# microsoft/EVA

Measured on AMD Instinct MI355X. Metric: homomorphic ops/sec (mul+rescale+relin) at N=2^16, L=10; execute() wall-time, higher is better.
Workload: dtype u64

## Files before the change

### eva_amd/csrc/internal.hip.h

```cpp
#pragma once
#include "../../include/eva_hip.h"

#include <hip/hip_runtime.h>

#include <algorithm>
#include <cmath>
#include <cstdlib>
#include <cstring>
#include <functional>
#include <map>
#include <memory>
#include <mutex>
#include <stdexcept>
#include <string>
#include <tuple>
#include <unordered_map>
#include <vector>

#include "devmath.hip.h"
#include "hostmath.h"

namespace evah {

extern thread_local std::string g_err;
// ... 36 lines not shown
    in_use += bytes;
    return p;
  }
  void free(void *p, size_t bytes) {
    bytes = (bytes + 255) & ~(size_t)255;
    free_[bytes].push_back(p);
    in_use -= bytes;
    cached += bytes;
  }
  void release_cached() {
    for (auto &kv : free_)
      for (void *p : kv.second) (void)hipFree(p);
    free_.clear();
    cached = 0;
  }
};

struct Buffer {
  u64 *d;
  size_t bytes;
  int refs;
  Pool *pool;
  evah_ctx *owner;
  bool ready_everywhere;
  std::vector<evah_ctx *> synced;
  std::vector<evah_ctx *> readers;
};

enum KClass {
  KC_EW = 0,
  KC_INTT_A,
  KC_INTT_B,
  KC_KSDIGIT_A,
  KC_KSDIGIT_B,
  KC_KSMAC,
  KC_MODDOWN_A,
  KC_MODDOWN_B,
  KC_NTT_A,
  KC_NTT_B,
  KC_COUNT
};
static const char *const kclass_names[KC_COUNT] = {
    "elementwise", "intt_pass1", "intt_pass2", "ksdigit_pass1", "ksdigit_pass2", "ks_mac",
    "moddown_pass1", "moddown_pass2", "ntt_pass1", "ntt_pass2"};

struct ProfRec {
  hipEvent_t e0, e1;
  int cls;
};

__host__ __device__ inline size_t keyp_block_words(uint32_t nd) { return ((size_t)2 * nd + 1) * 256; }
struct KeyDev {
  u64 *d = nullptr;
  uint32_t n_digits = 0;
  size_t bytes = 0;
  uint32_t rows = 0;
  u64 *d_split = nullptr;
  u64 *d_perm = nullptr;
};

}

using namespace evah;

struct evah_ct {
  Buffer *buf;
  u64 *d;
  uint32_t size, limbs;
  size_t ps;
  double scale;
  uint32_t batch = 1;
};
struct evah_pt {
  Buffer *buf;
  u64 *d;
  uint32_t limbs;
  double scale;
  bool uniform = false;
};
struct evah_graph {
  hipGraph_t graph = nullptr;
  hipGraphExec_t exec = nullptr;
  struct Reserved { evah_ctx *ctx; void *p; size_t bytes; };
  std::vector<Reserved> reserved;
};

struct SharedDev {
  int device = 0;
  void *d_tables = nullptr;
  KeyDev relin;
  KeyDev pk, sk;
  double2 *dec_roots = nullptr;
  std::map<uint32_t, KeyDev> galois;
  std::map<uint32_t, uint32_t *> perms;
  std::map<uint32_t, uint32_t *> perms_inv;
  std::map<uint32_t, u64 *> hoist_sign;
  std::map<std::pair<uint32_t, uint32_t>, u64 *> hoist_corr;
  double2 *enc_roots = nullptr;
  double enc_last_root[2] = {0, 0};
  uint32_t *enc_slot_map = nullptr;
  uint32_t key_rows = 0, key_shard = 0;
  uint64_t xfer[6] = {0, 0, 0, 0, 0, 0};
  ~SharedDev() {
    (void)hipSetDevice(device);
    if (enc_roots) (void)hipFree(enc_roots);
    if (enc_slot_map) (void)hipFree(enc_slot_map);
    if (relin.d) (void)hipFree(relin.d);
    if (relin.d_split) (void)hipFree(relin.d_split);
    if (pk.d) (void)hipFree(pk.d);
    if (sk.d) { (void)hipMemset(sk.d, 0, sk.bytes); (void)hipFree(sk.d); }
    if (dec_roots) (void)hipFree(dec_roots);
    for (auto &kv : galois) {
      (void)hipFree(kv.second.d);
      if (kv.second.d_split) (void)hipFree(kv.second.d_split);
      if (kv.second.d_perm) (void)hipFree(kv.second.d_perm);
    }
    for (auto &kv : perms) (void)hipFree(kv.second);
    for (auto &kv : perms_inv) (void)hipFree(kv.second);
    for (auto &kv : hoist_sign) (void)hipFree(kv.second);
    for (auto &kv : hoist_corr) (void)hipFree(kv.second);
    if (d_tables) (void)hipFree(d_tables);
  }
};

struct Tunables {
  bool fuse_mac = true;
  bool fuse_mul = true;
  bool fuse_mul2 = true;
  bool ew_fuse = true;
  bool ew_uniform = true;
  uint32_t fuse_small_blocks = 2048;
  int small_lr = 2;
  uint32_t small_lr_blocks = 1024;
  bool hoist = true;
  uint32_t hoist_min_tiles = 2048;
  bool hoist_debug = false;
  bool peer_self_check = false;
  bool hoist_table_fail = false;
  bool fuse_special_inv = true;
  int ks_groups = 1;
  int ks_threads = 64;
  bool fold_pa = true;
  bool win_fuse = true;
  bool win_linear = true;
  bool fb_persist = true;
  uint32_t fb_grid = 0;
  bool mac3 = true;
  uint32_t loop_n = 8, loop_min = 2, loop_min_wgs = 2048, loop_target_wgs = 8192;
  bool hoist_map = true;
  uint32_t hoist_v = 1;
  bool side_stream = false;
  bool chain_step = true, chain_batched = true;
  uint32_t chain_fuse_blocks = 256;
  uint32_t lds_extra = 0;

  static Tunables from_env(uint32_t N) {
    Tunables t;
    auto flag = [](const char *name, bool &v) { if (const char *e = std::getenv(name)) v = std::atoi(e) != 0; };
    auto count = [](const char *name, uint32_t &v) { if (const char *e = std::getenv(name)) v = (uint32_t)std::max(0, std::atoi(e)); };
    (void)N;
    flag("EVAH_FUSE_MAC", t.fuse_mac);
    flag("EVAH_FUSE_MUL", t.fuse_mul);
    flag("EVAH_FUSE_MUL2", t.fuse_mul2);
    flag("EVAH_EW_FUSE", t.ew_fuse);
    flag("EVAH_EW_UNIFORM", t.ew_uniform);
    count("EVAH_FUSE_SMALL", t.fuse_small_blocks);
    if (const char *e = std::getenv("EVAH_SMALL_LR")) t.small_lr = std::atoi(e) == 3 ? 3 : 2;
    count("EVAH_SMALL_LR_BLOCKS", t.small_lr_blocks);
    flag("EVAH_HOIST", t.hoist);
    count("EVAH_HOIST_MIN_TILES", t.hoist_min_tiles);
    flag("EVAH_HOIST_DEBUG", t.hoist_debug);
    flag("EVAH_HOIST_TABLE_FAIL", t.hoist_table_fail);
    flag("EVAH_PEER_SELF_CHECK", t.peer_self_check);
    flag("EVAH_FUSE_SPECIAL_INV", t.fuse_special_inv);
    flag("EVAH_FOLD_PA", t.fold_pa);
    flag("EVAH_WIN_FUSE", t.win_fuse);
    flag("EVAH_WIN_LINEAR", t.win_linear);
    flag("EVAH_FB_PERSIST", t.fb_persist);
    count("EVAH_FB_GRID", t.fb_grid);
    flag("EVAH_MAC3", t.mac3);
    count("EVAH_LOOP_N", t.loop_n);
    count("EVAH_LOOP_MIN", t.loop_min);
    count("EVAH_LOOP_MIN_WGS", t.loop_min_wgs);
    count("EVAH_LOOP_TARGET_WGS", t.loop_target_wgs);
    count("EVAH_LDS_EXTRA", t.lds_extra);
    flag("EVAH_HOIST_MAP", t.hoist_map);
    flag("EVAH_SIDE_STREAM", t.side_stream);
    flag("EVAH_CHAIN_STEP", t.chain_step);
    flag("EVAH_CHAIN_BATCHED", t.chain_batched);
    count("EVAH_CHAIN_FUSE_BLOCKS", t.chain_fuse_blocks);
    count("EVAH_HOIST_V", t.hoist_v);
    if (const char *e = std::getenv("EVAH_KS_GROUPS")) t.ks_groups = std::max(1, std::atoi(e));
    if (const char *e = std::getenv("EVAH_KS_THREADS")) {
      const int n = std::atoi(e);
      if (n == 64 || n == 128 || n == 256) t.ks_threads = n;
    }
    return t;
  }
};

struct evah_ctx {
  std::shared_ptr<SharedDev> sh;
  int device = 0;
  uint32_t N = 0, logN = 0, k = 0;
  std::vector<u64> primes;
  std::vector<int> total_bits;
  DevCtx dev{};
  hipStream_t own = nullptr, stream = nullptr;
  hipStream_t side = nullptr;
  Pool pool;
  hipEvent_t ev0 = nullptr, ev1 = nullptr;
  bool capturing = false;
  std::vector<hipEvent_t> capture_events;
  std::vector<hipEvent_t> sync_events;
  Tunables tun;
  bool all_tb = false;
  bool prof_on = false;
  std::vector<ProfRec> prof_recs;
  std::vector<hipEvent_t> prof_free;
  double prof_ms[KC_COUNT] = {0};
  uint64_t prof_n[KC_COUNT] = {0};
};

namespace evah {

inline void use(evah_ctx *c) { HIPCHK(hipSetDevice(c->device)); }
inline void count_h2d(evah_ctx *c, size_t bytes, bool plain = false) { c->sh->xfer[plain ? 2 : 0]++; c->sh->xfer[4] += bytes; }
inline void count_d2h(evah_ctx *c, size_t bytes, bool plain = false) { c->sh->xfer[plain ? 3 : 1]++; c->sh->xfer[5] += bytes; }

inline hipEvent_t prof_event(evah_ctx *c) {
  if (!c->prof_free.empty()) {
    hipEvent_t e = c->prof_free.back();
    c->prof_free.pop_back();
    return e;
  }
  hipEvent_t e;
  HIPCHK(hipEventCreate(&e));
  return e;
}
inline void prof_drain(evah_ctx *c) {
  for (auto &r : c->prof_recs) {
    float ms = 0;
    HIPCHK(hipEventSynchronize(r.e1));
    HIPCHK(hipEventElapsedTime(&ms, r.e0, r.e1));
    c->prof_ms[r.cls] += ms;
    c->prof_n[r.cls]++;
    c->prof_free.push_back(r.e0);
    c->prof_free.push_back(r.e1);
  }
  c->prof_recs.clear();
}
struct ProfScope {
  evah_ctx *c;
  int cls;
  hipEvent_t e0 = nullptr;
  ProfScope(evah_ctx *c_, int cls_) : c(c_), cls(cls_) {
    if (c->prof_on && !c->capturing) {
      if (c->prof_recs.size() >= 8192) prof_drain(c);
      e0 = prof_event(c);
      HIPCHK(hipEventRecord(e0, c->stream));
    }
  }
  ~ProfScope() {
    if (e0) {
      hipEvent_t e1 = prof_event(c);
      (void)hipEventRecord(e1, c->stream);
      c->prof_recs.push_back({e0, e1, cls});
    }
  }
};

inline Buffer *buf_new(evah_ctx *c, size_t elems) {
  Buffer *b = new Buffer;
  b->bytes = elems * sizeof(u64);
  b->d = (u64 *)c->pool.alloc(b->bytes);
  b->refs = 1;
  b->pool = &c->pool;
  b->owner = c;
  b->ready_everywhere = false;
  return b;
}
inline void h2d_now(evah_ctx *c, void *dst, const void *src, size_t bytes) {
  HIPCHK(hipMemcpyAsync(dst, src, bytes, hipMemcpyHostToDevice, c->stream));
  HIPCHK(hipStreamSynchronize(c->stream));
}
inline hipEvent_t sync_event(evah_ctx *c) {
  if (!c->capturing && !c->sync_events.empty()) {
    hipEvent_t e = c->sync_events.back();
    c->sync_events.pop_back();
    return e;
  }
  hipEvent_t e;
  HIPCHK(hipEventCreateWithFlags(&e, hipEventDisableTiming));
  return e;
}
inline void stream_wait(evah_ctx *waiter, evah_ctx *signaller) {
  if (waiter == signaller || waiter->stream == signaller->stream) return;
  if (waiter->sh.get() != signaller->sh.get()) {
    int cur = 0;
    HIPCHK(hipGetDevice(&cur));
    HIPCHK(hipSetDevice(signaller->device));
    hipEvent_t e = sync_event(signaller);
    hipError_t rc = hipEventRecord(e, signaller->stream);
    (void)hipSetDevice(waiter->device);
    if (rc == hipSuccess) rc = hipStreamWaitEvent(waiter->stream, e, 0);
    (void)hipSetDevice(cur);
    if (waiter->capturing || signaller->capturing) signaller->capture_events.push_back(e);
    else signaller->sync_events.push_back(e);
    HIPCHK(rc);
    return;
  }
  hipEvent_t e = sync_event(waiter);
  HIPCHK(hipEventRecord(e, signaller->stream));
  HIPCHK(hipStreamWaitEvent(waiter->stream, e, 0));
  if (waiter->capturing || signaller->capturing) waiter->capture_events.push_back(e);
  else waiter->sync_events.push_back(e);
}
struct SideStream {
  evah_ctx *c;
  hipStream_t main;
  bool forked = false, on_side = false;
  explicit SideStream(evah_ctx *c_) : c(c_), main(c_->stream) {}
  void link(hipStream_t from, hipStream_t to) {
    hipEvent_t e = sync_event(c);
    HIPCHK(hipEventRecord(e, from));
    HIPCHK(hipStreamWaitEvent(to, e, 0));
    if (c->capturing) c->capture_events.push_back(e);
    else c->sync_events.push_back(e);
  }
  void fork() {
    if (!c->side) HIPCHK(hipStreamCreateWithFlags(&c->side, hipStreamNonBlocking));
    link(main, c->side);
    c->stream = c->side;
    forked = on_side = true;
  }
  void back() { c->stream = main; on_side = false; }
  void join() {
    back();
    if (forked) link(c->side, main);
    forked = false;
  }
  ~SideStream() {
    c->stream = main;
// ... 108 lines not shown
```

### eva_amd/csrc/keyswitch.hip

```cpp
#include "launch.hip.h"

namespace evah {

__global__ void __launch_bounds__(256)
k_ks_mac(DevCtx cx, const u64 *target, const u64 *scratch, const u64 *key, u64 *prod, uint32_t l) {
  if (cx.skipped()) return;
  const uint32_t I = blockIdx.y;
  const uint32_t kap = (I == l) ? cx.k - 1 : I;
  const size_t n = 2 * ((size_t)blockIdx.x * blockDim.x + threadIdx.x);
  const DevPrime pm = cx.primes[kap];
  const size_t N = cx.N, key_digit = (size_t)2 * cx.k * N;
  u128_t a0x = {0, 0}, a0y = {0, 0}, a1x = {0, 0}, a1y = {0, 0};
  for (uint32_t J = 0; J < l; J++) {
    const u64 *op = (I == J) ? target + (size_t)J * N : scratch + ((size_t)I * l + J) * N;
    const ulonglong2 o = ld2(op + n);
    const u64 *kp = key + J * key_digit + (size_t)kap * N + n;
    const ulonglong2 k0 = ld2(kp), k1 = ld2(kp + (size_t)cx.k * N);
    acc128(a0x, o.x, k0.x);
    acc128(a0y, o.y, k0.y);
    acc128(a1x, o.x, k1.x);
    acc128(a1y, o.y, k1.y);
  }
  ulonglong2 r0, r1;
  r0.x = barrett128(a0x, pm);
  r0.y = barrett128(a0y, pm);
  r1.x = barrett128(a1x, pm);
  r1.y = barrett128(a1y, pm);
  st2(prod + (size_t)I * N + n, r0);
  st2(prod + ((size_t)(l + 1) + I) * N + n, r1);
}

template <int P, int LR>
static void launch_ks_inner_plr(evah_ctx *c, const u64 *target, const u64 *scratch, const KsBatch &kb, u64 *prod, uint32_t l) {
  ProfScope ps(c, KC_KSMAC);
  const uint32_t max_tile = (uint32_t)c->tun.ks_threads << LR;
  const uint32_t tile = c->N < max_tile ? c->N : max_tile;
  const int logC = (int)ilog2(tile) - P;
  if (logC < 0) throw std::runtime_error("ks_inner tile smaller than one sub-transform");
  const size_t lds = ((((size_t)1 << logC) * lds_sub_stride<P>() + 1) & ~(size_t)1) * sizeof(u64) +
                     ((size_t)1 << (logC + P)) * sizeof(ulonglong2) +
                     (kb.mac3 ? (size_t)tile * sizeof(u64) : 0);
  const uint32_t n_tiles = c->N / tile;
  auto go = [&](auto kernel, const auto &mt, const auto &at) {
    hipLaunchKernelGGL(kernel, dim3(n_tiles * kb.n, kb.ni), dim3(tile >> LR), lds, c->stream, c->dev, target, kb.target_bs, scratch,
                       kb.scratch_bs, kb.keys, prod, kb.prod_bs, l, kb.i0, logC, n_tiles, kb.n, kb.targets, mt, kb.istep,
                       kb.nout ? kb.nout : l + 1, kb.r_out, at, (kb.lazy_out ? 1 : 0) | (kb.diag ? 2 : 0), kb.fold_row);
  };
  if (kb.r_out && ((tile >> LR) > 64 || kb.istep != 1)) throw std::logic_error("fused special-row inverse pass needs the one-wave key-switch kernel");
  if (kb.fold && kb.istep != 1) throw std::logic_error("the folded key-switch forms are not used on limb shards");
  if (kb.fold && !kb.mul && !kb.adds) throw std::logic_error("folded key switch without polynomials to fold");
  const int mode = kb.mul ? (kb.fold ? KS_FOLDMUL : KS_MUL) : (kb.fold ? KS_FOLDADD : KS_PLAIN);
  auto with_mode = [&](auto mode_tag) {
    constexpr int M = decltype(mode_tag)::value;
    const KsMulArg<M> mt = [&] { if constexpr (M == KS_MUL || M == KS_FOLDMUL) return *kb.mul; else return NoMul{}; }();
    const KsAddArg<M> at = [&] { if constexpr (M == KS_FOLDADD) return *kb.adds; else return NoMul{}; }();
    if constexpr (M != KS_MUL) {
      if (kb.mac3 && (tile >> LR) <= 64) {
        if (kb.r_out) go(ks_inner_kernel<P, LR, 64, M, true, true>, mt, at);
        else go(ks_inner_kernel<P, LR, 64, M, false, true>, mt, at);
        return;
      }
    }
    if (kb.mac3) throw std::logic_error("split keys handed to a key-switch kernel that accumulates in 128 bits");
    if (kb.r_out) go(ks_inner_kernel<P, LR, 64, M, true>, mt, at);
    else if ((tile >> LR) <= 64) go(ks_inner_kernel<P, LR, 64, M>, mt, at);
    else go(ks_inner_kernel<P, LR, NTT_THREADS, M>, mt, at);
  };
  switch (mode) {
  case KS_PLAIN: with_mode(std::integral_constant<int, KS_PLAIN>{}); break;
  case KS_MUL: with_mode(std::integral_constant<int, KS_MUL>{}); break;
  case KS_FOLDMUL: with_mode(std::integral_constant<int, KS_FOLDMUL>{}); break;
  default: with_mode(std::integral_constant<int, KS_FOLDADD>{}); break;
  }
  HIPCHK(hipGetLastError());
}
template <int LR>
static void launch_ks_inner_lr(evah_ctx *c, int P, const u64 *target, const u64 *scratch, const KsBatch &key, u64 *prod, uint32_t l) {
  switch (P) {
  case 5: launch_ks_inner_plr<5, LR>(c, target, scratch, key, prod, l); break;
  case 6: launch_ks_inner_plr<6, LR>(c, target, scratch, key, prod, l); break;
  case 7: launch_ks_inner_plr<7, LR>(c, target, scratch, key, prod, l); break;
  case 8: launch_ks_inner_plr<8, LR>(c, target, scratch, key, prod, l); break;
  default: throw std::runtime_error("unsupported poly_modulus_degree for the key-switch kernel");
  }
}
void launch_ks_inner(evah_ctx *c, int P, const u64 *target, const u64 *scratch, const KsBatch &key, u64 *prod, uint32_t l) {
  launch_ks_inner_lr<2>(c, P, target, scratch, key, prod, l);
}

bool switch_key_products(evah_ctx *c, uint32_t l, const u64 *target, size_t target_bs, const KeyDev *const *keys,
                         uint32_t n, u64 *prod_d, const PtrTab *target_tab, const MulTab *mul, u64 *r_small, bool fold,
                         const PtrTab *adds, bool lazy_out) {
  const size_t N = c->N;
  if (n < 1 || n > (uint32_t)KS_BATCH_MAX) throw std::runtime_error("key-switch batch out of range");
  KsBatch kb;
  kb.n = n;
  kb.target_bs = target_bs;
  kb.scratch_bs = (size_t)(l + 1) * l * N;
  kb.prod_bs = (size_t)2 * (l + 1) * N;
  const uint32_t ks_tile = std::min<uint32_t>(c->N, (uint32_t)c->tun.ks_threads << 2);
  bool mac3 = c->tun.mac3 && c->tun.fuse_mac && c->all_tb && l <= 15 && (ks_tile >> 2) <= 64 && !(mul && !fold);
  for (uint32_t b = 0; b < n; b++) {
    if (keys[b]->n_digits < l) throw std::runtime_error("key switching key has too few digits");
    if (keys[b]->rows != c->k) throw std::logic_error("this context holds a limb shard's key rows: use the evah_shard_* entry points");
    mac3 = mac3 && keys[b]->d_split;
  }
  for (uint32_t b = 0; b < n; b++) kb.keys.key[b] = mac3 ? keys[b]->d_split : keys[b]->d;
  kb.mac3 = mac3;
  if (target_tab) kb.targets = *target_tab;
  kb.mul = mul;
  kb.fold = fold;
  kb.adds = adds;
  kb.lazy_out = lazy_out;
  if ((mul || fold) && !c->tun.fuse_mac) throw std::logic_error("the fused multiply / folded forms need the fused key-switch kernel");
  Scratch t(c, (size_t)n * l * N);
  Scratch sc(c, n * kb.scratch_bs);
  Scratch d2(c, mul && fold ? (size_t)n * l * N : 1);
  if (mul && fold) {
    target = d2.d;
    kb.target_bs = target_bs = (size_t)l * N;
  }
  OpKsDigit::Params dp{t.d, sc.d, l, (size_t)l * N, kb.scratch_bs, 0, l + 1};
  const bool small = c->tun.fuse_mac && std::max(1, c->tun.ks_groups) == 1 && fuse_small_launch(c, n * (l + 1) * l);
  if (mul) {
    OpMulIntt::Params ip{*mul, t.d, (size_t)l * N, l, fold ? d2.d : nullptr};
    if (small) launch_pass_p<false, true, OpMulIntt>(c, c->logN / 2, ip, n * l);
    else ntt_inverse<OpMulIntt>(c, ip, n * l);
  } else {
    OpPlain::Params ip{target, t.d, target_bs, (size_t)l * N, l, 0, 0, {}};
    if (target_tab) ip.src_tab = *target_tab;
    if (small) launch_pass_p<false, true, OpPlain>(c, c->logN / 2, ip, n * l);
    else ntt_inverse<OpPlain>(c, ip, n * l);
  }
  if (small) {
    dp.i0 = kb.i0 = 0;
    dp.ni = kb.ni = l + 1;
    launch_inv_fwd<OpKsDigit>(c, dp, n * (l + 1) * l);
    const uint32_t max_tile = (uint32_t)c->tun.ks_threads << 2;
    if (r_small && c->tun.fuse_special_inv && (std::min<uint32_t>(c->N, max_tile) >> 2) <= 64) kb.r_out = r_small;
    launch_ks_inner(c, c->logN / 2, target, sc.d, kb, prod_d, l);
    return kb.r_out != nullptr;
  }
  if (c->tun.fuse_mac) {
    const int a = (c->logN + 1) / 2, b = c->logN / 2;
    const uint32_t groups = std::min<uint32_t>(std::max(1, c->tun.ks_groups), l + 1);
    const uint32_t max_tile = (uint32_t)c->tun.ks_threads << 2;
    if (r_small && groups == 1 && c->tun.fuse_special_inv && (std::min<uint32_t>(c->N, max_tile) >> 2) <= 64) kb.r_out = r_small;
    for (uint32_t g = 0; g < groups; g++) {
      const uint32_t i0 = (uint32_t)((uint64_t)(l + 1) * g / groups), i1 = (uint32_t)((uint64_t)(l + 1) * (g + 1) / groups);
      if (i1 == i0) continue;
      dp.i0 = kb.i0 = i0;
      dp.ni = kb.ni = i1 - i0;
      launch_pass_p<true, false, OpKsDigit>(c, a, dp, n * (i1 - i0) * l);
      launch_ks_inner(c, b, target, sc.d, kb, prod_d, l);
    }
    return kb.r_out != nullptr;
  } else {
    ntt_forward<OpKsDigit>(c, dp, n * (l + 1) * l);
    for (uint32_t b = 0; b < n; b++) {
      ProfScope ps(c, KC_KSMAC);
      hipLaunchKernelGGL(k_ks_mac, dim3(c->N / 512, l + 1), dim3(256), 0, c->stream, c->dev,
                         target ? target + b * target_bs : target_tab->p[b], sc.d + b * kb.scratch_bs, keys[b]->d,
                         prod_d + b * kb.prod_bs, l);
      HIPCHK(hipGetLastError());
    }
  }
  return false;
}

void switch_key(evah_ctx *c, uint32_t l, const u64 *target, const KeyDev &key, const u64 *add,
                       size_t add_ps, uint32_t add_polys, u64 *out, size_t out_ps) {
  const size_t N = c->N;
  Scratch prod(c, (size_t)2 * (l + 1) * N);
  Scratch r(c, 2 * N);
  const KeyDev *kp = &key;
  const bool fold = c->tun.fold_pa && c->tun.fuse_mac && add && add_polys >= 1 && add_polys <= 2;
  PtrTab adds{};
  if (fold)
    for (uint32_t K = 0; K < add_polys; K++) adds.p[K] = add + K * add_ps;
  const bool inv1 = switch_key_products(c, l, target, 0, &kp, 1, prod.d, nullptr, nullptr, fuse_small_launch(c, 2 * l) ? r.d : nullptr,
                                        fold, fold ? &adds : nullptr);
  if (fold) add = nullptr;
  OpPlain::Params sp{prod.d + (size_t)l * N, r.d, (size_t)(l + 1) * N, N, 1, c->k - 1, 1, {}};
    OpModDown::Params mp{r.d, N, prod.d, (size_t)(l + 1) * N, add, add_ps, add_polys, out, out_ps,
                       c->k - 1, l};
  inverse_then_forward<OpPlain, OpModDown>(c, sp, 2, mp, 2 * l, inv1);
}

}

extern "C" {

int evah_relinearize(evah_ctx *c, const evah_ct *a, evah_ct **out) {
  API_BEGIN
  use(c);
  acquire(c, a->buf);
  if (a->size != 3) throw std::invalid_argument("relinearize expects a size-3 ciphertext");
  if (!c->sh->relin.d) throw std::invalid_argument("relinearization key not present");
  evah_ct *o = ct_new(c, 2, a->limbs, a->scale, a->batch);
  try {
    if (a->batch == 1) {
      switch_key(c, a->limbs, a->d + 2 * a->ps, c->sh->relin, a->d, a->ps, 2, o->d, o->ps);
    } else {
      const uint32_t l = a->limbs;
      const size_t N = c->N, pps = (size_t)(l + 1) * N;
      for (uint32_t b0 = 0; b0 < a->batch; b0 += KS_BATCH_MAX) {
        const uint32_t n = std::min<uint32_t>(KS_BATCH_MAX, a->batch - b0);
        const u64 *a0 = a->d + (size_t)b0 * 3 * a->ps;
        Scratch prod(c, (size_t)n * 2 * pps);
        std::vector<const KeyDev *> keys(n, &c->sh->relin);
        const bool fold = c->tun.fold_pa && c->tun.fuse_mac;
        PtrTab adds{};
        for (uint32_t b = 0; b < n && fold; b++)
          for (uint32_t K = 0; K < 2; K++) adds.p[2 * b + K] = a0 + (size_t)b * 3 * a->ps + K * a->ps;
        switch_key_products(c, l, a0 + 2 * a->ps, 3 * a->ps, keys.data(), n, prod.d, nullptr, nullptr, nullptr, fold, fold ? &adds : nullptr);
        Scratch r(c, (size_t)n * 2 * N);
        OpPlain::Params sp{prod.d + (size_t)l * N, r.d, pps, N, 1, c->k - 1, 1, {}};
        OpModDown::Params mp{r.d, N, prod.d, pps, fold ? nullptr : a0, a->ps, 2, o->d + (size_t)b0 * 2 * o->ps, o->ps, c->k - 1, l};
        mp.add_bs = 3 * a->ps;
        inverse_then_forward<OpPlain, OpModDown>(c, sp, 2 * n, mp, 2 * n * l);
      }
    }
  } catch (...) {
    evah_ct_free(c, o);
    throw;
  }
  *out = o;
  API_END
}

static void relin_rescale_core(evah_ctx *c, const evah_ct *const *as, uint32_t n, u64 *out_d, const MulTab *mul = nullptr,
                               uint32_t mul_limbs = 0);

int evah_relinearize_rescale(evah_ctx *c, const evah_ct *a, uint32_t divisor_bits, evah_ct **out) {
  API_BEGIN
  use(c);
  acquire(c, a->buf);
  if (a->size != 3) throw std::invalid_argument("relinearize expects a size-3 ciphertext");
  if (!c->sh->relin.d) throw std::invalid_argument("relinearization key not present");
  if (a->limbs < 2) throw std::invalid_argument("end of modulus switching chain reached");
  const uint32_t l = a->limbs, last = l - 1, sp = c->k - 1;
  const size_t N = c->N, pps = (size_t)(l + 1) * N;
  evah_ct *o = ct_new(c, 2, l - 1, a->scale / std::pow(2.0, (double)divisor_bits), a->batch);
  if (a->batch > 1) {
    try {
      std::vector<evah_ct> views(a->batch, *a);
      std::vector<const evah_ct *> ptrs(a->batch);
      for (uint32_t b = 0; b < a->batch; b++) {
        views[b].d = a->d + (size_t)b * 3 * a->ps;
        views[b].batch = 1;
        ptrs[b] = &views[b];
      }
      for (uint32_t b0 = 0; b0 < a->batch; b0 += KS_BATCH_MAX)
        relin_rescale_core(c, ptrs.data() + b0, std::min<uint32_t>(KS_BATCH_MAX, a->batch - b0),
                           o->d + (size_t)b0 * 2 * o->ps);
    } catch (...) {
      evah_ct_free(c, o);
      throw;
    }
    *out = o;
    g_err.clear();
    return 0;
  }
  try {
    Scratch prod(c, 2 * pps);
    const KeyDev *kp = &c->sh->relin;
    const bool fold = c->tun.fold_pa && c->tun.fuse_mac;
    PtrTab adds{};
    adds.p[0] = a->d;
    adds.p[1] = a->d + a->ps;
    switch_key_products(c, l, a->d + 2 * a->ps, 0, &kp, 1, prod.d, nullptr, nullptr, nullptr, fold, fold ? &adds : nullptr, fold);
    Scratch r(c, 2 * N), t(c, 2 * N);
    OpPlain::Params spp{prod.d + (size_t)l * N, r.d, pps, N, 1, sp, 1, {}};
    ntt_inverse<OpPlain>(c, spp, 2);
    if (fold) {
      OpRRLastFolded::Params lp{nullptr, 0, prod.d + (size_t)last * N, pps, r.d, N, t.d, N, last, sp, {}};
      ntt_inverse<OpRRLastFolded>(c, lp, 2);
      OpRRFolded::Params rp{r.d, N, t.d, N, nullptr, 0, prod.d, pps, o->d, o->ps, sp, last, l - 1, {}};
      ntt_forward<OpRRFolded>(c, rp, 2 * (l - 1));
    } else {
      OpRRLast::Params lp{a->d + (size_t)last * N, a->ps, prod.d + (size_t)last * N, pps, r.d, N, t.d, N, last, sp, {}};
      ntt_inverse<OpRRLast>(c, lp, 2);
      OpRR::Params rp{r.d, N, t.d, N, a->d, a->ps, prod.d, pps, o->d, o->ps, sp, last, l - 1, {}};
      ntt_forward<OpRR>(c, rp, 2 * (l - 1));
    }
  } catch (...) {
    evah_ct_free(c, o);
    throw;
  }
  *out = o;
  API_END
}

static void relin_rescale_core(evah_ctx *c, const evah_ct *const *as, uint32_t n, u64 *out_d, const MulTab *mul, uint32_t mul_limbs) {
  const uint32_t l = mul ? mul_limbs : as[0]->limbs;
  const uint32_t last = l - 1, sp = c->k - 1;
  const size_t N = c->N, pps = (size_t)(l + 1) * N, ops = (size_t)(l - 1) * N;
  PtrTab c2{}, a_last{}, a_polys{};
  for (uint32_t b = 0; b < n && !mul; b++) {
    const evah_ct *a = as[b];
    c2.p[b] = a->d + 2 * a->ps;
    for (uint32_t K = 0; K < 2; K++) {
      a_last.p[2 * b + K] = a->d + K * a->ps + (size_t)last * N;
      a_polys.p[2 * b + K] = a->d + K * a->ps;
    }
  }
// ... 497 lines not shown
```

### eva_amd/csrc/launch.hip.h

```cpp
#pragma once
#include "internal.hip.h"
#include "ntt.hip.h"

namespace evah {

#define EW_SETUP                                                                                 \
  const uint32_t p = blockIdx.z, i = blockIdx.y;                                                 \
  const size_t off = (size_t)i * cx.N + 2 * ((size_t)blockIdx.x * blockDim.x + threadIdx.x);    \
  const DevPrime pm = cx.primes[cx.prime_of(i)];                                                 \
  (void)p;                                                                                        \
  (void)pm;

__device__ __forceinline__ ulonglong2 ld2(const u64 *p) { return *reinterpret_cast<const ulonglong2 *>(p); }
__device__ __forceinline__ void st2(u64 *p, ulonglong2 v) { *reinterpret_cast<ulonglong2 *>(p) = v; }

template <class Op> struct OpClass;
template <bool Z, bool G> struct OpClass<OpPlainT<Z, G>> { static constexpr int fwd_a = KC_NTT_A, fwd_b = KC_NTT_B; };
template <> struct OpClass<OpMulIntt> { static constexpr int fwd_a = KC_NTT_A, fwd_b = KC_NTT_B; };
template <> struct OpClass<OpKsDigit> { static constexpr int fwd_a = KC_KSDIGIT_A, fwd_b = KC_KSDIGIT_B; };
template <bool G> struct OpClass<OpModDownT<G>> { static constexpr int fwd_a = KC_MODDOWN_A, fwd_b = KC_MODDOWN_B; };
template <> struct OpClass<OpMulPolyIntt> { static constexpr int fwd_a = KC_NTT_A, fwd_b = KC_NTT_B; };
template <> struct OpClass<OpModDownMul> { static constexpr int fwd_a = KC_MODDOWN_A, fwd_b = KC_MODDOWN_B; };
template <int M> struct OpClass<OpRRT<M>> { static constexpr int fwd_a = KC_MODDOWN_A, fwd_b = KC_MODDOWN_B; };
template <int M> struct OpClass<OpRRLastT<M>> { static constexpr int fwd_a = KC_MODDOWN_A, fwd_b = KC_MODDOWN_B; };
template <> struct OpClass<OpChainIntt> { static constexpr int fwd_a = KC_NTT_A, fwd_b = KC_NTT_B; };
template <> struct OpClass<OpChainT> { static constexpr int fwd_a = KC_INTT_B, fwd_b = KC_INTT_B; };
template <> struct OpClass<OpChainDigit> { static constexpr int fwd_a = KC_KSDIGIT_A, fwd_b = KC_KSDIGIT_B; };
template <> struct OpClass<OpRsMd> { static constexpr int fwd_a = KC_MODDOWN_A, fwd_b = KC_MODDOWN_B; };

template <int P, int LR, bool STRIDED, bool INVERSE, class Op>
static void launch_pass(evah_ctx *c, const typename Op::Params &prm, uint32_t jobs) {
  ProfScope ps(c, INVERSE ? (STRIDED ? KC_INTT_B : KC_INTT_A)
                          : (STRIDED ? OpClass<Op>::fwd_a : OpClass<Op>::fwd_b));
  const uint32_t max_tile = (uint32_t)NTT_THREADS << LR;
  const uint32_t tile = c->N < max_tile ? c->N : max_tile;
  const int logC = (int)ilog2(tile) - P;
  size_t lds = ((((size_t)1 << logC) * lds_sub_stride<P>() + 1) & ~(size_t)1) * sizeof(u64);
  if (STRIDED) lds += ((size_t)1 << P) * sizeof(ulonglong2);
  lds += c->tun.lds_extra;
  const uint32_t n_tiles = c->N / tile;
  const int log_tiles = (int)ilog2(n_tiles);
  dim3 grid = Op::grid(prm, jobs), block(tile >> LR);
  grid.x *= n_tiles;
  if (tile == max_tile) {
    hipLaunchKernelGGL((ntt_pass_kernel<P, LR, STRIDED, INVERSE, Op, true>), grid, block, lds, c->stream, c->dev,
                       prm, logC, log_tiles);
  } else if constexpr (P == 5) {
    hipLaunchKernelGGL((ntt_pass_kernel<P, LR, STRIDED, INVERSE, Op, false>), grid, block, lds, c->stream, c->dev,
                       prm, logC, log_tiles);
  } else {
    throw std::logic_error("partial NTT tile with P != 5");
  }
  HIPCHK(hipGetLastError());
}

template <int LR, bool STRIDED, bool INVERSE, class Op>
static void launch_pass_lr(evah_ctx *c, int P, const typename Op::Params &prm, uint32_t jobs) {
  switch (P) {
  case 5: launch_pass<5, LR, STRIDED, INVERSE, Op>(c, prm, jobs); break;
  case 6: launch_pass<6, LR, STRIDED, INVERSE, Op>(c, prm, jobs); break;
  case 7: launch_pass<7, LR, STRIDED, INVERSE, Op>(c, prm, jobs); break;
  case 8: launch_pass<8, LR, STRIDED, INVERSE, Op>(c, prm, jobs); break;
  case 9:
    if constexpr (STRIDED) { launch_pass<9, LR, STRIDED, INVERSE, Op>(c, prm, jobs); break; }
    [[fallthrough]];
  default: throw std::runtime_error("unsupported poly_modulus_degree for the NTT kernels");
  }
}
template <int P, bool INVERSE, class Op>
static bool launch_loop_pass(evah_ctx *c, const typename Op::Params &prm, uint32_t jobs) {
  constexpr int LR = 2;
  dim3 grid = Op::grid(prm, jobs);
  uint32_t ext[3] = {grid.x, grid.y, grid.z};
  const uint32_t count = ext[Op::loop_axis];
  if (!c->tun.loop_n || count < c->tun.loop_min || c->N < 256) return false;
  if ((uint64_t)ext[0] * ext[1] * ext[2] / count * (c->N / 256) * ((count + 1) / 2) < c->tun.loop_min_wgs) return false;
  ProfScope ps(c, INVERSE ? KC_INTT_A : OpClass<Op>::fwd_b);
  const uint32_t tile = 256, n_tiles = c->N / tile;
  const int logC = 8 - P, log_tiles = (int)ilog2(n_tiles);
  uint32_t nloop = std::min<uint32_t>(c->tun.loop_n, count);
  const uint64_t others = (uint64_t)ext[0] * ext[1] * ext[2] / count * n_tiles;
  while (nloop > 2 && others * ((count + nloop - 1) / nloop) < c->tun.loop_target_wgs) nloop = (nloop + 1) / 2;
  ext[Op::loop_axis] = (count + nloop - 1) / nloop;
  const size_t lds = ((((size_t)1 << logC) * lds_sub_stride<P>() + 1) & ~(size_t)1) * sizeof(u64) +
                     ((size_t)1 << (logC + P)) * sizeof(ulonglong2);
  hipLaunchKernelGGL((ntt_loop_kernel<P, LR, INVERSE, Op>), dim3(ext[0] * n_tiles, ext[1], ext[2]), dim3(tile >> LR), lds, c->stream,
                     c->dev, prm, logC, log_tiles, nloop, count);
  HIPCHK(hipGetLastError());
  return true;
}
template <bool INVERSE, class Op>
static bool launch_loop_pass_p(evah_ctx *c, int P, const typename Op::Params &prm, uint32_t jobs) {
  switch (P) {
  case 5: return launch_loop_pass<5, INVERSE, Op>(c, prm, jobs);
  case 6: return launch_loop_pass<6, INVERSE, Op>(c, prm, jobs);
  case 7: return launch_loop_pass<7, INVERSE, Op>(c, prm, jobs);
  case 8: return launch_loop_pass<8, INVERSE, Op>(c, prm, jobs);
  default: return false;
  }
}

template <bool STRIDED, bool INVERSE, class Op>
static void launch_pass_p(evah_ctx *c, int P, const typename Op::Params &prm, uint32_t jobs) {
  if constexpr (!STRIDED) {
    if (launch_loop_pass_p<INVERSE, Op>(c, P, prm, jobs)) return;
  }
  if (c->tun.small_lr == 2 && (uint64_t)jobs * (c->N >> 11) <= c->tun.small_lr_blocks && c->N >= 2048) {
    launch_pass_lr<2, STRIDED, INVERSE, Op>(c, P, prm, jobs);
    return;
  }
  launch_pass_lr<3, STRIDED, INVERSE, Op>(c, P, prm, jobs);
}

struct KsBatch {
  uint32_t n = 1;
  uint32_t i0 = 0, ni = 0;
  size_t target_bs = 0, scratch_bs = 0, prod_bs = 0;
  KsKeys keys{};
  PtrTab targets{};
  const MulTab *mul = nullptr;
  bool fold = false;
  const PtrTab *adds = nullptr;
  bool mac3 = false;
  bool lazy_out = false;
  uint32_t istep = 1, nout = 0;
  u64 *r_out = nullptr;
  bool diag = false;
  uint32_t fold_row = ~0u;
};
void launch_ks_inner(evah_ctx *c, int P, const u64 *target, const u64 *scratch, const KsBatch &key, u64 *prod, uint32_t l);

template <class Op> static void ntt_forward(evah_ctx *c, const typename Op::Params &prm, uint32_t jobs) {
  const int a = (c->logN + 1) / 2, b = c->logN / 2;
  launch_pass_p<true, false, Op>(c, a, prm, jobs);
  launch_pass_p<false, false, Op>(c, b, prm, jobs);
}
template <class Op> static void ntt_inverse(evah_ctx *c, const typename Op::Params &prm, uint32_t jobs) {
  const int a = (c->logN + 1) / 2, b = c->logN / 2;
  launch_pass_p<false, true, Op>(c, b, prm, jobs);
  launch_pass_p<true, true, Op>(c, a, prm, jobs);
}

static inline bool fuse_small_launch(evah_ctx *c, uint32_t fwd_jobs) {
  const uint32_t tile = (uint32_t)NTT_THREADS << 3;
  if (!c->tun.fuse_small_blocks || c->N < tile) return false;
  if (c->dev.guard) return true;
  return (uint64_t)fwd_jobs * (c->N / tile) <= c->tun.fuse_small_blocks;
}
template <int P, class Op, int LR> static void launch_inv_fwd_plr(evah_ctx *c, const typename Op::Params &prm, uint32_t jobs) {
  ProfScope ps(c, OpClass<Op>::fwd_a);
  const uint32_t tile = (uint32_t)NTT_THREADS << LR, n_tiles = c->N / tile;
  const int logC = (int)ilog2(tile) - P;
  const size_t lds = ((((size_t)1 << logC) * lds_sub_stride<P>() + 1) & ~(size_t)1) * sizeof(u64) + 2 * ((size_t)1 << P) * sizeof(ulonglong2);
  dim3 grid = Op::grid(prm, jobs);
  grid.x *= n_tiles;
  hipLaunchKernelGGL((ntt_inv_fwd_kernel<P, LR, Op>), grid, dim3(NTT_THREADS), lds, c->stream, c->dev, prm, (int)ilog2(n_tiles));
  HIPCHK(hipGetLastError());
}
template <int P, class Op> static void launch_inv_fwd_p(evah_ctx *c, const typename Op::Params &prm, uint32_t jobs) {
  if (c->tun.small_lr == 2) launch_inv_fwd_plr<P, Op, 2>(c, prm, jobs);
  else launch_inv_fwd_plr<P, Op, 3>(c, prm, jobs);
}
template <class Op> static void launch_inv_fwd(evah_ctx *c, const typename Op::Params &prm, uint32_t jobs) {
  switch ((c->logN + 1) / 2) {
  case 6: launch_inv_fwd_p<6, Op>(c, prm, jobs); break;
  case 7: launch_inv_fwd_p<7, Op>(c, prm, jobs); break;
  case 8: launch_inv_fwd_p<8, Op>(c, prm, jobs); break;
  case 9: launch_inv_fwd_p<9, Op>(c, prm, jobs); break;
  default: throw std::runtime_error("unsupported poly_modulus_degree for the fused inverse/forward pass");
  }
}
template <int P, class Op, bool FWD, int LR> static void launch_inv2_plr(evah_ctx *c, const typename Op::Params &prm, uint32_t jobs) {
  ProfScope ps(c, OpClass<Op>::fwd_a);
  const uint32_t tile = (uint32_t)NTT_THREADS << LR, n_tiles = c->N / tile;
  const int logC = (int)ilog2(tile) - P;
  const size_t lds = ((((size_t)1 << logC) * lds_sub_stride<P>() + 1) & ~(size_t)1) * sizeof(u64) + 2 * ((size_t)1 << P) * sizeof(ulonglong2);
  dim3 grid = Op::grid(prm, jobs);
  grid.x *= n_tiles;
  hipLaunchKernelGGL((ntt_inv2_kernel<P, LR, Op, FWD>), grid, dim3(NTT_THREADS), lds, c->stream, c->dev, prm, (int)ilog2(n_tiles));
  HIPCHK(hipGetLastError());
}
template <class Op, bool FWD> static void launch_inv2(evah_ctx *c, const typename Op::Params &prm, uint32_t jobs) {
  auto go = [&](auto ptag) {
    constexpr int P = decltype(ptag)::value;
    if (c->tun.small_lr == 2) launch_inv2_plr<P, Op, FWD, 2>(c, prm, jobs);
    else launch_inv2_plr<P, Op, FWD, 3>(c, prm, jobs);
  };
  switch ((c->logN + 1) / 2) {
  case 6: go(std::integral_constant<int, 6>{}); break;
  case 7: go(std::integral_constant<int, 7>{}); break;
  case 8: go(std::integral_constant<int, 8>{}); break;
  case 9: go(std::integral_constant<int, 9>{}); break;
  default: throw std::runtime_error("unsupported poly_modulus_degree for the fused inverse/forward pass");
  }
}
template <class InvOp, class Op>
static void inverse_then_forward(evah_ctx *c, const typename InvOp::Params &ip, uint32_t inv_jobs, const typename Op::Params &fp,
                                 uint32_t fwd_jobs, bool inv_pass1_done = false) {
  if (inv_pass1_done && !fuse_small_launch(c, fwd_jobs)) throw std::logic_error("fused inverse pass outside the small-launch form");
  if (fuse_small_launch(c, fwd_jobs)) {
    if (!inv_pass1_done) launch_pass_p<false, true, InvOp>(c, c->logN / 2, ip, inv_jobs);
    launch_inv_fwd<Op>(c, fp, fwd_jobs);
    launch_pass_p<false, false, Op>(c, c->logN / 2, fp, fwd_jobs);
  } else {
    ntt_inverse<InvOp>(c, ip, inv_jobs);
    ntt_forward<Op>(c, fp, fwd_jobs);
  }
}

bool switch_key_products(evah_ctx *c, uint32_t l, const u64 *target, size_t target_bs, const KeyDev *const *keys, uint32_t n,
                         u64 *prod_d, const PtrTab *target_tab = nullptr, const MulTab *mul = nullptr, u64 *r_small = nullptr,
                         bool fold = false, const PtrTab *adds = nullptr, bool lazy_out = false);
void switch_key(evah_ctx *c, uint32_t l, const u64 *target, const KeyDev &key, const u64 *add, size_t add_ps, uint32_t add_polys,
                u64 *out, size_t out_ps);
void key_split_launch(evah_ctx *c, const u64 *src, u64 *dst, size_t words);
const uint32_t *perm_table(evah_ctx *c, uint32_t elt);
void galois_perm_launch(evah_ctx *c, const u64 *a, size_t a_ps, uint32_t limbs, uint32_t polys, const uint32_t *perm, u64 *out, size_t o_ps);
void enc_tables(evah_ctx *c);

}
```

### eva_amd/csrc/ntt.hip.h

```cpp
#pragma once
#ifndef EVAH_DIGIT_AUX
#define EVAH_DIGIT_AUX 0
#endif
#include "devmath.hip.h"
#include <type_traits>

namespace evah {


constexpr int NTT_THREADS = 256;
constexpr uint32_t HOIST_ZERO_CAP = 64;

template <int P, int LR> struct Rounds {
  static constexpr int NR = (P + LR - 1) / LR;
  static constexpr int bits(int i) { return P / NR + (i < P % NR ? 1 : 0); }
  static constexpr int lo(int i) {
    int l = P;
    for (int j = 0; j <= i; j++) l -= bits(j);
    return l;
  }
};

#ifndef EVAH_LDS_PAD2
#define EVAH_LDS_PAD2 1
// ... 321 lines not shown
  for (int idx = threadIdx.x; idx < (C << P); idx += T) {
    const int sb = idx >> P, n = idx & (S - 1);
    if (n) {
      const int d = 31 - __clz(n);
      twl[idx] = tw[((size_t)((1u << pre) + sub0 + sb) << d) + (n - (1 << d))];
    }
  }
  auto load_tile = [&](const typename Op::Job &jj, ulonglong2 *d) {
#pragma unroll
    for (int it = 0; it < NPAIR; it++) {
      const uint32_t n = gbase + 2 * (threadIdx.x + it * T);
      if constexpr (INVERSE) {
        d[it].x = Op::template load<false>(cx, jj, pm, n);
        d[it].y = Op::template load<false>(cx, jj, pm, n + 1);
      } else {
        d[it] = *reinterpret_cast<const ulonglong2 *>(jj.dst + n);
      }
    }
  };
  constexpr bool PREFETCH = EVAH_PREFETCH && !INVERSE && HasPre<Op>::value;
  constexpr bool LOOPPRE = EVAH_PREFETCH && !INVERSE && !PREFETCH && HasLoopPre<Op>::value;
  constexpr bool RAW = INVERSE && HasRaw<Op>::value;
  ulonglong2 dreg[NPAIR];
  typename RawOf<Op, RAW>::type raw[NTT_R];
  load_tile(jb, dreg);
  while (true) {
    typename Op::Job jn;
    uint32_t jnext = j + 1;
    while (jnext < j1 && !setup(jnext, jn)) jnext++;
    const bool more = jnext < j1;
    __syncthreads();
#pragma unroll
    for (int it = 0; it < NPAIR; it++) {
      const int idx = 2 * (threadIdx.x + it * T);
      const int sb = idx >> P, e = idx & (S - 1);
      lds[sb * SP + lds_pad<P>(e)] = dreg[it].x;
      lds[sb * SP + lds_pad<P>(e + 1)] = dreg[it].y;
    }
    typename PreOf<Op, PREFETCH>::type epi[NTT_R];
    if constexpr (PREFETCH) {
#pragma unroll
      for (int it = 0; it < NTT_R; it++) epi[it] = Op::prefetch(cx, jb, pm, gbase + 2 * (threadIdx.x + (it >> 1) * T) + (it & 1));
    }
    typename LoopPreOf<Op, LOOPPRE>::type lepi[NTT_R];
    if constexpr (LOOPPRE) {
#pragma unroll
      for (int it = 0; it < NTT_R; it++) lepi[it] = Op::loop_prefetch(cx, jb, pm, gbase + 2 * (threadIdx.x + (it >> 1) * T) + (it & 1));
    }
    if constexpr (RAW) {
      if (more) {
#pragma unroll
        for (int it = 0; it < NTT_R; it++) raw[it] = Op::raw_load(cx, jn, pm, gbase + 2 * (threadIdx.x + (it >> 1) * T) + (it & 1));
      }
    } else {
      if (more) load_tile(jn, dreg);
    }
    __syncthreads();
    if constexpr (INVERSE) RoundSeq<P, LR, 0, true, true, true, false>::run(lds + sub * SP, tid, 0, 0, twl + (sub << P), pm);
    else forward_rounds<P, LR, true, true>(lds + sub * SP, tid, 0, 0, twl + (sub << P), pm);
    __syncthreads();
#pragma unroll
    for (int it = 0; it < NPAIR; it++) {
      const int idx = 2 * (threadIdx.x + it * T);
      const int sb = idx >> P, e = idx & (S - 1);
      const uint32_t n = gbase + idx;
      const u64 vx = lds[sb * SP + lds_pad<P>(e)], vy = lds[sb * SP + lds_pad<P>(e + 1)];
      if constexpr (INVERSE) {
        ulonglong2 v;
        v.x = vx;
        v.y = vy;
        *reinterpret_cast<ulonglong2 *>(jb.dst + n) = v;
      } else if constexpr (PREFETCH) {
        Op::store_fwd_pre(cx, jb, pm, n, vx, epi[2 * it]);
        Op::store_fwd_pre(cx, jb, pm, n + 1, vy, epi[2 * it + 1]);
      } else if constexpr (LOOPPRE) {
        Op::store_fwd_loop(cx, jb, pm, n, vx, lepi[2 * it]);
        Op::store_fwd_loop(cx, jb, pm, n + 1, vy, lepi[2 * it + 1]);
      } else {
        Op::store_fwd(cx, jb, pm, n, vx);
        Op::store_fwd(cx, jb, pm, n + 1, vy);
      }
    }
    if (!more) break;
    if constexpr (RAW) {
#pragma unroll
      for (int it = 0; it < NPAIR; it++) {
        const uint32_t n = gbase + 2 * (threadIdx.x + it * T);
        dreg[it].x = Op::finish_load(cx, jn, pm, n, raw[2 * it]);
        dreg[it].y = Op::finish_load(cx, jn, pm, n + 1, raw[2 * it + 1]);
      }
    }
    jb = jn;
    j = jnext;
  }
}

template <int P, int LR, class Op>
__global__ void __launch_bounds__(NTT_THREADS)
ntt_inv_fwd_kernel(DevCtx cx, typename Op::Params prm, int log_tiles) {
  extern __shared__ __attribute__((aligned(16))) u64 lds[];
  constexpr int NTT_R = 1 << LR;
  constexpr int S = 1 << P, TPS = S / NTT_R, SP = lds_sub_stride<P>();
  if (cx.skipped()) return;
  const uint32_t tile_idx = blockIdx.x & ((1u << log_tiles) - 1u);
  typename Op::Job jb;
  if (!Op::setup(cx, prm, blockIdx.x >> log_tiles, blockIdx.y, blockIdx.z, jb)) return;
  const uint32_t pa = Op::pre_prime(prm, jb);
  const DevPrime pmA = cx.primes[pa], pm = cx.primes[jb.prime];
  const ulonglong2 *twA = cx.tw_inv + (size_t)pa * cx.N, *tw = cx.tw_fwd + (size_t)jb.prime * cx.N;
  constexpr int logC = 8 + LR - P, C = 1 << logC, T = NTT_THREADS;
  const uint32_t stride_log = cx.logN - P;
  constexpr int ES = 1 << (P - LR);
  constexpr bool LINEAR = (ES % 16 == 0);
  const int c = threadIdx.x & (C - 1), e0 = threadIdx.x >> logC;
  const uint32_t n0 = (tile_idx << logC) + ((uint32_t)e0 << stride_log) + c, nstep = (uint32_t)(T >> logC) << stride_log;
  const int l0 = c * SP + lds_pad<P>(e0);
  auto lds_at = [&](int it) -> int {
    if constexpr (LINEAR) return l0 + it * lds_pad<P>(ES);
    const int idx = threadIdx.x + it * T;
    return (idx & (C - 1)) * SP + lds_pad<P>(idx >> logC);
  };
  const u64 *src = Op::pre_src(jb);
#pragma unroll
  for (int it = 0; it < NTT_R; it++) lds[lds_at(it)] = src[n0 + it * nstep];
  ulonglong2 *twlA = reinterpret_cast<ulonglong2 *>(lds + ((C * SP + 1) & ~1)), *twl = twlA + S;
  for (int idx = threadIdx.x; idx < S; idx += T) { twlA[idx] = twA[idx]; twl[idx] = tw[idx]; }
  __syncthreads();
  const int sub = threadIdx.x / TPS, tid = threadIdx.x % TPS;
  RoundSeq<P, LR, 0, true, true, false>::run(lds + sub * SP, tid, 0, 0, twlA, pmA);
  __syncthreads();
  auto convert = [&](auto lazy_tag) {
    constexpr bool LZ = decltype(lazy_tag)::value;
#pragma unroll
    for (int it = 0; it < NTT_R; it++) {
      u64 v = lds[lds_at(it)];
      if (Op::pre_addhalf) v = addmod(v, pmA.q >> 1, pmA.q);
      lds[lds_at(it)] = Op::template conv<LZ>(jb, pm, v);
    }
  };
  if (jb.lazy) convert(std::true_type{});
  else convert(std::false_type{});
  __syncthreads();
  forward_rounds<P, LR, true, false>(lds + sub * SP, tid, 0, 0, twl, pm);
  __syncthreads();
#pragma unroll
  for (int it = 0; it < NTT_R; it++) jb.dst[n0 + it * nstep] = lds[lds_at(it)];
}

}

#include "ntt_window_sum.hip.h"
#include "ntt_ks_inner.hip.h"
#include "ntt_ops.hip.h"
#include "ntt_chain.hip.h"
```

Baseline: 14310.

## Add fused mod-up kernel reusing inverse-NTT digit across all target primes

Adds a mod-up kernel that loads each key-switch digit tile once, finishes its inverse NTT pass in LDS, then loops over every target prime, converting and running the forward pass while prefetching the next prime's twiddles into registers. The inverse pass in the non-small path now uses the single-pass form so the mod-up kernel can complete it. This replaces one first-pass launch per (digit, prime) job, removing redundant global reads and the repeated inverse work. In exchange each block does serial work over l+1 primes, which gives fewer blocks and less parallelism, and it applies only with ks_groups=1 and supported N.

```diff
diff --git a/eva_amd/csrc/internal.hip.h b/eva_amd/csrc/internal.hip.h
--- a/eva_amd/csrc/internal.hip.h
+++ b/eva_amd/csrc/internal.hip.h
@@ -212,6 +212,7 @@
   bool side_stream = false;
   bool chain_step = true, chain_batched = true;
   uint32_t chain_fuse_blocks = 256;
+  bool modup = true;
   uint32_t lds_extra = 0;
 
   static Tunables from_env(uint32_t N) {
@@ -249,6 +250,7 @@
     flag("EVAH_CHAIN_STEP", t.chain_step);
     flag("EVAH_CHAIN_BATCHED", t.chain_batched);
     count("EVAH_CHAIN_FUSE_BLOCKS", t.chain_fuse_blocks);
+    flag("EVAH_MODUP", t.modup);
     count("EVAH_HOIST_V", t.hoist_v);
     if (const char *e = std::getenv("EVAH_KS_GROUPS")) t.ks_groups = std::max(1, std::atoi(e));
     if (const char *e = std::getenv("EVAH_KS_THREADS")) {
diff --git a/eva_amd/csrc/keyswitch.hip b/eva_amd/csrc/keyswitch.hip
--- a/eva_amd/csrc/keyswitch.hip
+++ b/eva_amd/csrc/keyswitch.hip
@@ -122,14 +122,15 @@
   }
   OpKsDigit::Params dp{t.d, sc.d, l, (size_t)l * N, kb.scratch_bs, 0, l + 1};
   const bool small = c->tun.fuse_mac && std::max(1, c->tun.ks_groups) == 1 && fuse_small_launch(c, n * (l + 1) * l);
+  const bool modup = !small && c->tun.modup && c->tun.fuse_mac && std::max(1, c->tun.ks_groups) == 1 && modup_fits(c);
   if (mul) {
     OpMulIntt::Params ip{*mul, t.d, (size_t)l * N, l, fold ? d2.d : nullptr};
-    if (small) launch_pass_p<false, true, OpMulIntt>(c, c->logN / 2, ip, n * l);
+    if (small || modup) launch_pass_p<false, true, OpMulIntt>(c, c->logN / 2, ip, n * l);
     else ntt_inverse<OpMulIntt>(c, ip, n * l);
   } else {
     OpPlain::Params ip{target, t.d, target_bs, (size_t)l * N, l, 0, 0, {}};
     if (target_tab) ip.src_tab = *target_tab;
-    if (small) launch_pass_p<false, true, OpPlain>(c, c->logN / 2, ip, n * l);
+    if (small || modup) launch_pass_p<false, true, OpPlain>(c, c->logN / 2, ip, n * l);
     else ntt_inverse<OpPlain>(c, ip, n * l);
   }
   if (small) {
@@ -151,7 +152,8 @@
       if (i1 == i0) continue;
       dp.i0 = kb.i0 = i0;
       dp.ni = kb.ni = i1 - i0;
-      launch_pass_p<true, false, OpKsDigit>(c, a, dp, n * (i1 - i0) * l);
+      if (modup) launch_modup<OpKsDigit>(c, dp, n);
+      else launch_pass_p<true, false, OpKsDigit>(c, a, dp, n * (i1 - i0) * l);
       launch_ks_inner(c, b, target, sc.d, kb, prod_d, l);
     }
     return kb.r_out != nullptr;
diff --git a/eva_amd/csrc/launch.hip.h b/eva_amd/csrc/launch.hip.h
--- a/eva_amd/csrc/launch.hip.h
+++ b/eva_amd/csrc/launch.hip.h
@@ -170,6 +170,27 @@
   default: throw std::runtime_error("unsupported poly_modulus_degree for the fused inverse/forward pass");
   }
 }
+static inline bool modup_fits(evah_ctx *c) { return c->N >= ((uint32_t)NTT_THREADS << 3) && (c->logN + 1) / 2 <= 9; }
+template <int P, class Op> static void launch_modup_p(evah_ctx *c, const typename Op::Params &prm, uint32_t n) {
+  ProfScope ps(c, OpClass<Op>::fwd_a);
+  constexpr int LR = 3;
+  const uint32_t tile = (uint32_t)NTT_THREADS << LR, n_tiles = c->N / tile;
+  const int logC = (int)ilog2(tile) - P;
+  const size_t lds = ((((size_t)1 << logC) * lds_sub_stride<P>() + 1) & ~(size_t)1) * sizeof(u64) + ((size_t)1 << P) * sizeof(ulonglong2);
+  hipLaunchKernelGGL((ntt_modup_kernel<P, LR, Op>), dim3(n_tiles * prm.l, 1, n), dim3(NTT_THREADS), lds, c->stream, c->dev, prm,
+                     (int)ilog2(n_tiles));
+  HIPCHK(hipGetLastError());
+}
+template <class Op> static void launch_modup(evah_ctx *c, const typename Op::Params &prm, uint32_t n) {
+  if (!modup_fits(c) || prm.i0 != 0 || prm.istep != 1) throw std::logic_error("mod-up kernel outside its shapes");
+  switch ((c->logN + 1) / 2) {
+  case 6: launch_modup_p<6, Op>(c, prm, n); break;
+  case 7: launch_modup_p<7, Op>(c, prm, n); break;
+  case 8: launch_modup_p<8, Op>(c, prm, n); break;
+  case 9: launch_modup_p<9, Op>(c, prm, n); break;
+  default: throw std::runtime_error("unsupported poly_modulus_degree for the mod-up kernel");
+  }
+}
 template <int P, class Op, bool FWD, int LR> static void launch_inv2_plr(evah_ctx *c, const typename Op::Params &prm, uint32_t jobs) {
   ProfScope ps(c, OpClass<Op>::fwd_a);
   const uint32_t tile = (uint32_t)NTT_THREADS << LR, n_tiles = c->N / tile;
diff --git a/eva_amd/csrc/ntt.hip.h b/eva_amd/csrc/ntt.hip.h
--- a/eva_amd/csrc/ntt.hip.h
+++ b/eva_amd/csrc/ntt.hip.h
@@ -497,4 +497,5 @@
 #include "ntt_window_sum.hip.h"
 #include "ntt_ks_inner.hip.h"
 #include "ntt_ops.hip.h"
+#include "ntt_modup.hip.h"
 #include "ntt_chain.hip.h"
diff --git a/eva_amd/csrc/ntt_modup.hip.h b/eva_amd/csrc/ntt_modup.hip.h
--- /dev/null
+++ b/eva_amd/csrc/ntt_modup.hip.h
@@ -0,0 +1,85 @@
+#pragma once
+#include "ntt.hip.h"
+
+namespace evah {
+
+template <int P, int LR, class Op>
+__global__ void __launch_bounds__(NTT_THREADS)
+ntt_modup_kernel(DevCtx cx, typename Op::Params prm, int log_tiles) {
+  extern __shared__ __attribute__((aligned(16))) u64 lds[];
+  constexpr int NTT_R = 1 << LR;
+  constexpr int S = 1 << P, TPS = S / NTT_R, SP = lds_sub_stride<P>();
+  constexpr int logC = 8 + LR - P, C = 1 << logC, T = NTT_THREADS;
+  constexpr int TWR = (S + T - 1) / T;
+  if (cx.skipped()) return;
+  const uint32_t tile_idx = blockIdx.x & ((1u << log_tiles) - 1u), J = blockIdx.x >> log_tiles, b = blockIdx.z;
+  typename Op::Job jb;
+  uint32_t iy = 0;
+  while (iy < prm.ni && !Op::setup(cx, prm, J, iy, b, jb)) iy++;
+  if (iy >= prm.ni) return;
+  const uint32_t pa = Op::pre_prime(prm, jb);
+  const DevPrime pmA = cx.primes[pa];
+  const uint32_t stride_log = cx.logN - P;
+  constexpr int ES = 1 << (P - LR);
+  constexpr bool LINEAR = (ES % 16 == 0);
+  const int c = threadIdx.x & (C - 1), e0 = threadIdx.x >> logC;
+  const uint32_t n0 = (tile_idx << logC) + ((uint32_t)e0 << stride_log) + c, nstep = (uint32_t)(T >> logC) << stride_log;
+  const int l0 = c * SP + lds_pad<P>(e0);
+  auto lds_at = [&](int it) -> int {
+    if constexpr (LINEAR) return l0 + it * lds_pad<P>(ES);
+    const int idx = threadIdx.x + it * T;
+    return (idx & (C - 1)) * SP + lds_pad<P>(idx >> logC);
+  };
+  const u64 *src = Op::pre_src(jb);
+#pragma unroll
+  for (int it = 0; it < NTT_R; it++) lds[lds_at(it)] = src[n0 + it * nstep];
+  ulonglong2 *twl = reinterpret_cast<ulonglong2 *>(lds + ((C * SP + 1) & ~1));
+  const ulonglong2 *twA = cx.tw_inv + (size_t)pa * cx.N;
+  for (int idx = threadIdx.x; idx < S; idx += T) twl[idx] = twA[idx];
+  ulonglong2 twn[TWR];
+  auto tw_request = [&](uint32_t prime) {
+    const ulonglong2 *tw = cx.tw_fwd + (size_t)prime * cx.N;
+#pragma unroll
+    for (int r = 0; r < TWR; r++)
+      if (S >= T || (int)threadIdx.x + r * T < S) twn[r] = tw[threadIdx.x + r * T];
+  };
+  tw_request(jb.prime);
+  __syncthreads();
+  const int sub = threadIdx.x / TPS, tid = threadIdx.x % TPS;
+  RoundSeq<P, LR, 0, true, true, false>::run(lds + sub * SP, tid, 0, 0, twl, pmA);
+  __syncthreads();
+  u64 t[NTT_R];
+#pragma unroll
+  for (int it = 0; it < NTT_R; it++) {
+    t[it] = lds[lds_at(it)];
+    if (Op::pre_addhalf) t[it] = addmod(t[it], pmA.q >> 1, pmA.q);
+  }
+  while (true) {
+#pragma unroll
+    for (int r = 0; r < TWR; r++)
+      if (S >= T || (int)threadIdx.x + r * T < S) twl[threadIdx.x + r * T] = twn[r];
+    const DevPrime pm = cx.primes[jb.prime];
+    auto convert = [&](auto lazy_tag) {
+      constexpr bool LZ = decltype(lazy_tag)::value;
+#pragma unroll
+      for (int it = 0; it < NTT_R; it++) lds[lds_at(it)] = Op::template conv<LZ>(jb, pm, t[it]);
+    };
+    if (jb.lazy) convert(std::true_type{});
+    else convert(std::false_type{});
+    typename Op::Job jn;
+    uint32_t in = iy + 1;
+    while (in < prm.ni && !Op::setup(cx, prm, J, in, b, jn)) in++;
+    const bool more = in < prm.ni;
+    if (more) tw_request(jn.prime);
+    __syncthreads();
+    forward_rounds<P, LR, true, false>(lds + sub * SP, tid, 0, 0, twl, pm);
+    __syncthreads();
+#pragma unroll
+    for (int it = 0; it < NTT_R; it++) jb.dst[n0 + it * nstep] = lds[lds_at(it)];
+    if (!more) break;
+    jb = jn;
+    iy = in;
+  }
+}
+
+}
```

New measurement: 14890, median of 6. +4.1%, better.
